# sea-sky-web/Vision-based-Spatio-Temporal-Analysis

Hardware: AMD Instinct MI355X
Metric: multi-cam frames/sec (7-cam→480×1440 BEV) (higher is better)
Workload: dtype f32; 1 GPU; 7-cam 1080x1920 -> resnet50(stride-8 features)+proj C=64 -> IPM warp -> mean -> 480x1440 BEV (BASELINE configs[1]); cameras=7, cameras_per_gpu=7, channels=64, bev_memory_format=NCHW, parallelism=frame-sharded x1 (no collective)

## Files before the change

### vision-based-spatio-temporal-analysis_amd/csrc/bev_conv_x6.hip

```cpp
#include <hip/hip_runtime.h>
#include <stdint.h>

#include <type_traits>

#include "../../include/bev_mi355x.h"
#include "bev_act.h"

namespace {

typedef __bf16 bf16x8 __attribute__((ext_vector_type(8)));
typedef __bf16 bf16x4 __attribute__((ext_vector_type(4)));
typedef float f32x16 __attribute__((ext_vector_type(16)));
typedef float f32x4 __attribute__((ext_vector_type(4)));
typedef unsigned u32x4 __attribute__((ext_vector_type(4)));
typedef unsigned u32x2 __attribute__((ext_vector_type(2)));

constexpr int XBK = 16;
constexpr int XROW = 24;

__device__ __attribute__((aligned(16))) float g_xzero4[4] = {0.f, 0.f, 0.f, 0.f};

__host__ __device__ inline int64_t kpad_x(int K) { return (K + XBK - 1) / XBK * XBK; }
__host__ __device__ inline int64_t copad_x(int Co) { return (Co + 127) / 128 * 128; }

// ... 650 lines not shown
        _Pragma("unroll") for (int i = 0; i < TM; ++i)                                                     \
            _Pragma("unroll") for (int p = 0; p < 3; ++p)                                                  \
                fa[i][p] = *(const bf16x8 *)(AS + p * APL + (wm * TM * 32 + i * 32 + r32) * YROW + 16 * (KK) + 8 * h); \
        _Pragma("unroll") for (int i = 0; i < TM; ++i)                                                     \
            _Pragma("unroll") for (int j = 0; j < TN; ++j) {                                               \
                acc[i][j] = __builtin_amdgcn_mfma_f32_32x32x16_bf16(fa[i][0], BC[j][0], acc[i][j], 0, 0, 0); \
                acc[i][j] = __builtin_amdgcn_mfma_f32_32x32x16_bf16(fa[i][0], BC[j][1], acc[i][j], 0, 0, 0); \
                acc[i][j] = __builtin_amdgcn_mfma_f32_32x32x16_bf16(fa[i][1], BC[j][0], acc[i][j], 0, 0, 0); \
                acc[i][j] = __builtin_amdgcn_mfma_f32_32x32x16_bf16(fa[i][0], BC[j][2], acc[i][j], 0, 0, 0); \
                acc[i][j] = __builtin_amdgcn_mfma_f32_32x32x16_bf16(fa[i][2], BC[j][0], acc[i][j], 0, 0, 0); \
                acc[i][j] = __builtin_amdgcn_mfma_f32_32x32x16_bf16(fa[i][1], BC[j][1], acc[i][j], 0, 0, 0); \
            }                                                                                              \
    } while (0)
#define X6B_MFMA(BUF, KS)                                                                                  \
    do {                                                                                                   \
        const __bf16 *As = lds + (BUF) * STAGE;                                                            \
        X6B_SLICE(As, 0, bs0);                                                                             \
        X6B_BLOAD(bs0, 2 * (KS) + 2);                                                                      \
        X6B_SLICE(As, 1, bs1);                                                                             \
    } while (0)

    const int nk = a.Kp / YBK;
    X6B_BLOAD(bs0, 0);
    X6B_GLOAD(va0);
    if (nk > 1) X6B_GLOAD(va1);
    X6B_SWRITE(0, va0);
    __syncthreads();
    int ks = 0;
    for (; ks + 3 < nk; ks += 2) {
        X6B_BLOAD(bs1, 2 * ks + 1);
        X6B_GLOAD(va0);
        X6B_MFMA(0, ks);
        X6B_SWRITE(1, va1);
        __syncthreads();
        X6B_BLOAD(bs1, 2 * ks + 3);
        X6B_GLOAD(va1);
        X6B_MFMA(1, ks + 1);
        X6B_SWRITE(0, va0);
        __syncthreads();
    }
    if (ks + 2 < nk) {
        X6B_BLOAD(bs1, 2 * ks + 1);
        X6B_GLOAD(va0);
        X6B_MFMA(0, ks);
        X6B_SWRITE(1, va1);
        __syncthreads();
        X6B_BLOAD(bs1, 2 * ks + 3);
        X6B_MFMA(1, ks + 1);
        X6B_SWRITE(0, va0);
        __syncthreads();
        X6B_BLOAD(bs1, 2 * ks + 5);
        X6B_MFMA(0, ks + 2);
    } else if (ks + 1 < nk) {
        X6B_BLOAD(bs1, 2 * ks + 1);
        X6B_MFMA(0, ks);
        X6B_SWRITE(1, va1);
        __syncthreads();
        X6B_BLOAD(bs1, 2 * ks + 3);
        X6B_MFMA(1, ks + 1);
    } else {
        X6B_BLOAD(bs1, 2 * ks + 1);
        X6B_MFMA(0, ks);
    }
#undef X6B_MFMA
#undef X6B_SLICE
#undef X6B_BLOAD
#undef X6B_SWRITE
#undef X6B_GLOAD
    if constexpr (CHAIN > 0) {
        x6_chain_epilogue<WM, WN, TM, TN, CHAIN == 2 ? 4 : 0>(a, lds_raw, acc, wave, lane, wm, wn, m0);
        return;
    }
    x6_epilogue<TM, TN>(a, (float *)lds_raw, acc, wave, lane, wn, wm, m0, n0);
}

template <int WM, int WN, int TM, int TN, int CHAIN = 0>
__global__ __launch_bounds__(256, CHAIN ? 2 : 3) void k_conv_x6s(ConvX a) {
    constexpr bool BLDS = CHAIN > 0;
    constexpr int BM = WM * TM * 32, BN = WN * TN * 32;
    constexpr int APL = BM * 32;
    constexpr int BST = BLDS ? BN / 32 * 6 * 512 : 0;
    constexpr int STAGE = 3 * APL + BST;
    constexpr int RW = BM / 4;
    constexpr int RG = RW / 16;
    constexpr int BPW = BLDS ? BN / 32 * 6 / 4 : 0;
    constexpr int EPIB = CHAIN ? x6_chain_lds_bytes<BM, BN>() : x6_epi_bytes<TN>();
    constexpr int LDSB = (2 * STAGE * 2 > EPIB) ? 2 * STAGE * 2 : EPIB;
    static_assert(RW % 16 == 0, "whole DMA groups per wave");
    static_assert(!BLDS || (BN / 32 * 6) % 4 == 0, "whole B pieces per wave");
    __shared__ __attribute__((aligned(16))) unsigned char lds_raw[LDSB];
    const __bf16 *lds = (const __bf16 *)lds_raw;

    const int tid = threadIdx.x;
    const int lane = tid & 63, wave = __builtin_amdgcn_readfirstlane(tid >> 6);
    const int wm = wave / WN, wn = wave % WN;
    const int n_tiles = (a.Co + BN - 1) / BN;
    unsigned bid = blockIdx.x;
    {
        const unsigned nb = gridDim.x, q = nb / 8, r = nb % 8, xc = bid % 8;
        bid = (xc < r ? xc * (q + 1) : r * (q + 1) + (xc - r) * q) + bid / 8;
    }
    const int64_t m0 = (int64_t)(bid / n_tiles) * BM;
    const int n0 = (bid % n_tiles) * BN;

    int64_t abase[RG];
    int aiy[RG], aix[RG];
    bool aok[RG];
#pragma unroll
    for (int g = 0; g < RG; ++g) {
        const int row = wave * RW + 16 * g + (lane >> 2);
        const int lc = (lane & 3) ^ ((row >> 2) & 3);
        const int64_t m = m0 + row;
        aok[g] = m < a.M;
        const int64_t mm = aok[g] ? m : 0;
        const int ox = (int)(mm % a.Wo);
        const int64_t t = mm / a.Wo;
        const int oy = (int)(t % a.Ho);
        const int64_t n = t / a.Ho;
        aiy[g] = oy * a.stride - a.pad;
        aix[g] = ox * a.stride - a.pad;
        abase[g] = ((n * a.H + aiy[g]) * a.W + aix[g]) * a.Ci + 8 * lc;
    }
    const unsigned lbase = (unsigned)__builtin_amdgcn_readfirstlane((int)lds_addr(lds_raw));
    const int S = a.Kp / XBK;
    int ky = 0, kx = 0, ci0 = 0, kstep = 0;
    const __bf16 *bsrc = a.wp + (int64_t)(n0 >> 5) * S * 1536 + lane * 8;
    auto issue = [&](int buf) {
        if constexpr (BLDS) {
            const unsigned db = lbase + (unsigned)(buf * STAGE * 2 + 3 * APL * 2);
#pragma unroll
            for (int i = 0; i < BPW; ++i) {
                const int q = wave + 4 * i, cbl = q / 6, r = q % 6;
                dma16(bsrc + ((int64_t)cbl * S + 2 * kstep + r / 3) * 1536 + (r % 3) * 512,
                      db + (unsigned)(q * 1024));
            }
            ++kstep;
        }
        const int64_t toff = ((int64_t)ky * a.dil * a.W + kx * a.dil) * a.Ci + ci0;
        const unsigned d0 = lbase + (unsigned)(buf * STAGE * 2) + (unsigned)(wave * RW * 64);
#pragma unroll
        for (int g = 0; g < RG; ++g) {
            const int iy = aiy[g] + ky * a.dil, ix = aix[g] + kx * a.dil;
            const bool in = aok[g] && (unsigned)iy < (unsigned)a.H && (unsigned)ix < (unsigned)a.W;
            const __bf16 *src = a.xs + abase[g] + toff;
#pragma unroll
            for (int p = 0; p < 3; ++p)
                dma16(in ? (const void *)(src + p * a.xps) : (const void *)g_xzero4,
                      d0 + (unsigned)(p * APL * 2 + g * 1024));
        }
        ci0 += YBK;
        if (ci0 == a.Ci) {
            ci0 = 0;
            if (++kx == a.KW) {
                kx = 0;
                ++ky;
            }
        }
    };

    const __amdgpu_buffer_rsrc_t rw = __builtin_amdgcn_make_buffer_rsrc(
        const_cast<__bf16 *>(a.wp), 0, (int)(uint32_t)(copad_x(a.Co) / 32 * (int64_t)S * 3072), 0x00020000);
    const int cb0 = (n0 + wn * TN * 32) >> 5;
    const int vl = lane * 16;
    bf16x8 bs0[TN][3], bs1[TN][3];
#define X6S_BLOAD(BS, G)                                                                                   \
    do {                                                                                                   \
        const int g_ = (G) < S ? (G) : S - 1;                                                              \
        _Pragma("unroll") for (int j = 0; j < TN; ++j)                                                     \
            _Pragma("unroll") for (int p = 0; p < 3; ++p)                                                  \
                BS[j][p] = __builtin_bit_cast(                                                             \
                    bf16x8, __builtin_amdgcn_raw_buffer_load_b128(rw, vl, (((cb0 + j) * S + g_) * 3 + p) * 1024, 0)); \
    } while (0)
    const int r32 = lane & 31, h = lane >> 5;
#define X6S_SLICE(AS, KK, BC)                                                                              \
    do {                                                                                                   \
        bf16x8 fa[TM][3];                                                                                  \
        _Pragma("unroll") for (int i = 0; i < TM; ++i) {                                                   \
            const int R = wm * TM * 32 + i * 32 + r32;                                                     \
            const int ph = (2 * (KK) + h) ^ ((R >> 2) & 3);                                                \
            _Pragma("unroll") for (int p = 0; p < 3; ++p)                                                  \
                fa[i][p] = *(const bf16x8 *)(AS + p * APL + R * 32 + ph * 8);                              \
        }                                                                                                  \
        _Pragma("unroll") for (int i = 0; i < TM; ++i)                                                     \
            _Pragma("unroll") for (int j = 0; j < TN; ++j) {                                               \
                acc[i][j] = __builtin_amdgcn_mfma_f32_32x32x16_bf16(fa[i][0], BC[j][0], acc[i][j], 0, 0, 0); \
                acc[i][j] = __builtin_amdgcn_mfma_f32_32x32x16_bf16(fa[i][0], BC[j][1], acc[i][j], 0, 0, 0); \
                acc[i][j] = __builtin_amdgcn_mfma_f32_32x32x16_bf16(fa[i][1], BC[j][0], acc[i][j], 0, 0, 0); \
                acc[i][j] = __builtin_amdgcn_mfma_f32_32x32x16_bf16(fa[i][0], BC[j][2], acc[i][j], 0, 0, 0); \
                acc[i][j] = __builtin_amdgcn_mfma_f32_32x32x16_bf16(fa[i][2], BC[j][0], acc[i][j], 0, 0, 0); \
                acc[i][j] = __builtin_amdgcn_mfma_f32_32x32x16_bf16(fa[i][1], BC[j][1], acc[i][j], 0, 0, 0); \
            }                                                                                              \
    } while (0)

    f32x16 acc[TM][TN];
#pragma unroll
    for (int i = 0; i < TM; ++i)
#pragma unroll
        for (int j = 0; j < TN; ++j) acc[i][j] = (f32x16){0};
    const int nk = a.Kp / YBK;
    if constexpr (BLDS) {
        issue(0);
        asm volatile("s_waitcnt vmcnt(0)" ::: "memory");
        __syncthreads();
        for (int ks = 0; ks < nk; ++ks) {
            const int cur = ks & 1;
            if (ks + 1 < nk) issue(cur ^ 1);
            const __bf16 *As = lds + cur * STAGE;
            const __bf16 *Bs = As + 3 * APL + lane * 8;
#pragma unroll
            for (int kk = 0; kk < 2; ++kk) {
                bf16x8 fb[TN][3];
#pragma unroll
                for (int j = 0; j < TN; ++j)
#pragma unroll
                    for (int p = 0; p < 3; ++p) fb[j][p] = *(const bf16x8 *)(Bs + (((wn * TN + j) * 2 + kk) * 3 + p) * 512);
                X6S_SLICE(As, kk, fb);
            }
            asm volatile("s_waitcnt vmcnt(0)" ::: "memory");
            __syncthreads();
        }
    } else {
        X6S_BLOAD(bs0, 0);
        issue(0);
        asm volatile("s_waitcnt vmcnt(0)" ::: "memory");
        __syncthreads();
        for (int ks = 0; ks < nk; ++ks) {
            const int cur = ks & 1;
            if (ks + 1 < nk) issue(cur ^ 1);
            const __bf16 *As = lds + cur * STAGE;
            X6S_BLOAD(bs1, 2 * ks + 1);
            X6S_SLICE(As, 0, bs0);
            X6S_BLOAD(bs0, 2 * ks + 2);
            X6S_SLICE(As, 1, bs1);
            asm volatile("s_waitcnt vmcnt(0)" ::: "memory");
            __syncthreads();
        }
    }
#undef X6S_SLICE
#undef X6S_BLOAD
    if constexpr (CHAIN > 0) {
        x6_chain_epilogue<WM, WN, TM, TN, CHAIN == 2 ? 4 : 0>(a, lds_raw, acc, wave, lane, wm, wn, m0);
        return;
    }
    x6_epilogue<TM, TN>(a, (float *)lds_raw, acc, wave, lane, wn, wm, m0, n0);
}

__global__ void k_split3(const float *__restrict__ x, int64_t n, __bf16 *__restrict__ out) {
    const int64_t t = (int64_t)blockIdx.x * blockDim.x + threadIdx.x;
    if (t >= n) return;
    __bf16 h, m, l;
    split3(x[t], h, m, l);
    out[t] = h;
    out[t + n] = m;
    out[t + 2 * n] = l;
}

template <int BM, int BN>
int launch_x6(void (*kernel)(ConvX), const ConvX &a, hipStream_t st) {
    const int64_t blocks = ((a.M + BM - 1) / BM) * ((a.Co + BN - 1) / BN);
    if (blocks >= ((int64_t)1 << 31)) return BEV_ERR_ARGS;
    hipLaunchKernelGGL(kernel, dim3((unsigned)blocks), dim3(256), 0, st, a);
    return (int)hipGetLastError();
}

ConvX conv_x6_args(const float *x, const uint16_t *packed, const float *bias, const float *res, float *y, int N, int H,
                   int W, int Ci, int Co, int KH, int KW, int stride, int pad, int dil, int Ho, int Wo, int act,
                   int ldy) {
    ConvX a;
    a.x = x, a.wp = (const __bf16 *)packed, a.bias = bias, a.res = res, a.y = y;
    a.N = N, a.H = H, a.W = W, a.Ci = Ci, a.Co = Co, a.KH = KH, a.KW = KW, a.stride = stride, a.pad = pad;
    a.dil = dil, a.Ho = Ho, a.Wo = Wo, a.act = act, a.ldy = ldy;
    a.Kp = (int)kpad_x(Ci * KH * KW);
    a.M = (int64_t)N * Ho * Wo;
    return a;
}

int g_x6_tile = 0;
int g_x6_nt = 0;
int g_x6_kernel = 0;

template <bool DUAL>
int dispatch_x6(const ConvX &a0, hipStream_t st) {
    ConvX a = a0;
    a.nta = g_x6_nt;
    const int t = g_x6_tile ? g_x6_tile : (a.Co <= 64 ? 2 : 1);
    if (!DUAL && a.xs) {
        if (t == 2) return launch_x6<128, 64>(k_conv_x6s<4, 1, 1, 2>, a, st);
        return launch_x6<128, 128>(k_conv_x6s<2, 2, 2, 2>, a, st);
    }
    const bool wide = a.Ci % YBK == 0 && (!DUAL || a.Ci2 % YBK == 0) && g_x6_kernel != 1;
    if (wide) {
        if (t == 2 && !DUAL && a.nta) return launch_x6<128, 64>(k_conv_x6b<4, 1, 1, 2, false, 0, true>, a, st);
        if (t == 2) return launch_x6<128, 64>(k_conv_x6b<4, 1, 1, 2, DUAL>, a, st);
        return launch_x6<128, 128>(k_conv_x6b<2, 2, 2, 2, DUAL>, a, st);
    }
    if (t == 2) return launch_x6<128, 64>(k_conv_x6<4, 1, 1, 2, DUAL>, a, st);
    return launch_x6<128, 128>(k_conv_x6<2, 2, 2, 2, DUAL>, a, st);
}

namespace stem6 {
constexpr int TW = 64, TH = 8, NTHR = 512;
constexpr int PR = 2 * TH + 5;
constexpr int PC = 2 * TW + 5;
constexpr int PP = 80;
constexpr int RP = 2 * PP, CP = PR * RP, PATCH = 3 * CP;
constexpr int NE = 3 * PR * PC;
constexpr int PER_T = (NE + NTHR - 1) / NTHR;
constexpr int NS = 10;
constexpr int WB = 2 * NS * 3 * 512;
__host__ __device__ constexpr int koff(int k) {
    return k >= 147 ? 0 : (k % 3) * CP + (k / 21) * RP + (((k / 3) % 7) & 1) * PP + (((k / 3) % 7) >> 1);
}
}

struct StemX6Args {
    const float *__restrict__ x;
    const __bf16 *__restrict__ wp;
    const float *__restrict__ bias;
    float *__restrict__ y;
    int H, W, Co, Ho, Wo, relu, nTx, nTy;
    int64_t ntiles;
    float *__restrict__ edge_b, *__restrict__ edge_r;
    int Hp, Wp;
};

__device__ __forceinline__ void stem6_fetch(const StemX6Args &a, int64_t t, int tid, float (&pv)[stem6::PER_T]) {
    using namespace stem6;
    const int tx = (int)(t % a.nTx);
    const int64_t r_ = t / a.nTx;
    const int ty = (int)(r_ % a.nTy);
    const int64_t img = r_ / a.nTy;
    const int row0 = 2 * ty * TH - 3, col0 = 2 * tx * TW - 3;
    const float *xi = a.x + img * 3 * (int64_t)a.H * a.W;
#pragma unroll
    for (int i = 0; i < PER_T; ++i) {
        const int e = tid + NTHR * i;
        const int cr = e / PC, c = e - cr * PC;
        const int ci = cr / PR, r = cr - ci * PR;
        const int gy = row0 + r, gx = col0 + c;
        const bool in = e < NE && gy >= 0 && gy < a.H && gx >= 0 && gx < a.W;
        pv[i] = *(in ? xi + ((int64_t)ci * a.H + gy) * a.W + gx : (const float *)g_xzero4);
    }
}

__device__ __forceinline__ void stem6_put(float *pl, int tid, const float (&pv)[stem6::PER_T]) {
    using namespace stem6;
#pragma unroll
    for (int i = 0; i < PER_T; ++i) {
        const int e = tid + NTHR * i;
        if (e < NE) {
            const int cr = e / PC, c = e - cr * PC;
            const int ci = cr / PR, r = cr - ci * PR;
            const int o = ci * CP + r * RP + (c & 1) * PP + (c >> 1);
            __bf16 hh, mm, ll;
            split3(pv[i], hh, mm, ll);
            reinterpret_cast<unsigned *>(pl)[o] = (unsigned)__builtin_bit_cast(unsigned short, hh) |
                                                  ((unsigned)__builtin_bit_cast(unsigned short, mm) << 16);
            reinterpret_cast<__bf16 *>(pl + PATCH)[o] = ll;
        }
    }
}

__device__ __forceinline__ float pool_mx(float m, float v) { return max_nan(m, v); }

template <bool POOL>
__global__ __launch_bounds__(stem6::NTHR, 1) void k_stem_x6(StemX6Args a) {
    using namespace stem6;
    __shared__ __attribute__((aligned(16))) unsigned char lds_raw[WB * 2 + PATCH * 6];
    __bf16 *wl = (__bf16 *)lds_raw;
    float *pl = (float *)(lds_raw + WB * 2);
    const int tid = threadIdx.x, lane = tid & 63, wave = tid >> 6, h = lane >> 5, r32 = lane & 31;
    for (int e = tid; e < WB / 8; e += NTHR) reinterpret_cast<u32x4 *>(wl)[e] = reinterpret_cast<const u32x4 *>(a.wp)[e];
    float pv[PER_T];
    int64_t t = blockIdx.x;
    stem6_fetch(a, t < a.ntiles ? t : 0, tid, pv);
    stem6_put(pl, tid, pv);
    __syncthreads();

    const float *P = pl + wave * 2 * RP + r32;
    const __bf16 *PL = reinterpret_cast<const __bf16 *>(pl + PATCH) + wave * 2 * RP + r32;
    const float b0 = (r32 < a.Co) ? a.bias[r32] : 0.0f;
    const float b1 = (32 + r32 < a.Co) ? a.bias[32 + r32] : 0.0f;
    for (; t < a.ntiles; t += gridDim.x) {
        const int64_t tn = t + gridDim.x;
        stem6_fetch(a, tn < a.ntiles ? tn : t, tid, pv);
        f32x16 acc[2][2];
#pragma unroll
        for (int i = 0; i < 2; ++i)
#pragma unroll
            for (int j = 0; j < 2; ++j) acc[i][j] = (f32x16){0};
#pragma unroll
        for (int sl = 0; sl < NS; ++sl) {
            int hv = h;
            asm volatile("" : "+v"(hv));
            const __bf16 *wlb = wl + lane * 8;
            asm volatile("" : "+v"(wlb));
            bf16x8 fb[2][3];
#pragma unroll
            for (int j = 0; j < 2; ++j)
#pragma unroll
                for (int p = 0; p < 3; ++p)
                    fb[j][p] = *(const bf16x8 *)(wlb + ((j * NS + sl) * 3 + p) * 512);
#pragma unroll
            for (int mt = 0; mt < 2; ++mt) {
                bf16x8 fa[3];
#pragma unroll
                for (int e = 0; e < 8; ++e) {
                    const int o0 = koff(16 * sl + e), o1 = koff(16 * sl + 8 + e);
                    const int o = 32 * mt + (hv ? o1 : o0);
                    const unsigned hm = reinterpret_cast<const unsigned *>(P)[o];
                    fa[0][e] = __builtin_bit_cast(__bf16, (unsigned short)(hm & 0xffffu));
                    fa[1][e] = __builtin_bit_cast(__bf16, (unsigned short)(hm >> 16));
                    fa[2][e] = PL[o];
                }
#pragma unroll
                for (int j = 0; j < 2; ++j) {
                    f32x16 &c = acc[mt][j];
                    c = __builtin_amdgcn_mfma_f32_32x32x16_bf16(fa[0], fb[j][0], c, 0, 0, 0);
                    c = __builtin_amdgcn_mfma_f32_32x32x16_bf16(fa[0], fb[j][1], c, 0, 0, 0);
                    c = __builtin_amdgcn_mfma_f32_32x32x16_bf16(fa[1], fb[j][0], c, 0, 0, 0);
                    c = __builtin_amdgcn_mfma_f32_32x32x16_bf16(fa[0], fb[j][2], c, 0, 0, 0);
                    c = __builtin_amdgcn_mfma_f32_32x32x16_bf16(fa[2], fb[j][0], c, 0, 0, 0);
                    c = __builtin_amdgcn_mfma_f32_32x32x16_bf16(fa[1], fb[j][1], c, 0, 0, 0);
                }
            }
            __builtin_amdgcn_sched_barrier(0);
        }
        if constexpr (POOL) {
            const int tx = (int)(t % a.nTx);
            const int64_t r_ = t / a.nTx;
            const int ty = (int)(r_ % a.nTy);
            const int64_t img = r_ / a.nTy;
            const int oy = ty * TH + wave;
            const int oxb = tx * TW;
            float hp[2][4][2][2];
            float pa3[2][2][4];
            float c63[2];
#pragma unroll
            for (int mt = 0; mt < 2; ++mt)
#pragma unroll
                for (int j = 0; j < 2; ++j)
#pragma unroll
                    for (int b = 0; b < 4; ++b) {
                        float v[4];
#pragma unroll
                        for (int u = 0; u < 4; ++u) {
                            const int ox = oxb + 32 * mt + 8 * b + 4 * h + u;
                            const float z = acc[mt][j][4 * b + u] + (j ? b1 : b0);
                            v[u] = oy < a.Ho && ox < a.Wo ? relu_f(z) : 0.0f;
                        }
                        pa3[mt][j][b] = __shfl_xor(v[3], 32);
                        hp[mt][b][1][j] = pool_mx(pool_mx(v[1], v[2]), v[3]);
                        hp[mt][b][0][j] = pool_mx(v[0], v[1]);
                        if (mt == 1 && b == 3) c63[j] = v[3];
                    }
#pragma unroll
            for (int mt = 0; mt < 2; ++mt)
#pragma unroll
                for (int j = 0; j < 2; ++j)
#pragma unroll
                    for (int b = 0; b < 4; ++b) {
                        const float prev0 = b > 0 ? pa3[mt][j][b - 1] : (mt > 0 ? pa3[mt - 1][j][3] : 0.0f);
                        hp[mt][b][0][j] = pool_mx(hp[mt][b][0][j], h ? pa3[mt][j][b] : prev0);
                    }
            __syncthreads();
            float *xl = pl;
            if (wave & 1) {
                float *o = xl + (wave >> 1) * 34 * 64 + lane;
#pragma unroll
                for (int mt = 0; mt < 2; ++mt)
#pragma unroll
                    for (int b = 0; b < 4; ++b)
#pragma unroll
                        for (int pc = 0; pc < 2; ++pc)
#pragma unroll
                            for (int j = 0; j < 2; ++j) o[(((mt * 4 + b) * 2 + pc) * 2 + j) * 64] = hp[mt][b][pc][j];
                o[32 * 64] = c63[0];
                o[33 * 64] = c63[1];
            }
            __syncthreads();
            const int64_t tile = t;
            if (wave == TH - 1) {
                float *eb = a.edge_b + tile * (32 * 64);
#pragma unroll
                for (int mt = 0; mt < 2; ++mt)
#pragma unroll
                    for (int b = 0; b < 4; ++b)
#pragma unroll
                        for (int pc = 0; pc < 2; ++pc)
#pragma unroll
                            for (int j = 0; j < 2; ++j)
                                eb[(16 * mt + 4 * b + 2 * h + pc) * 64 + r32 + 32 * j] = hp[mt][b][pc][j];
                if (h) {
                    a.edge_r[(tile * 5 + 4) * 64 + r32] = c63[0];
                    a.edge_r[(tile * 5 + 4) * 64 + 32 + r32] = c63[1];
                }
            } else if (!(wave & 1)) {
                const int p = wave >> 1;
                const float *up = xl + (p - 1) * 34 * 64 + lane, *dn = xl + p * 34 * 64 + lane;
#pragma unroll
                for (int mt = 0; mt < 2; ++mt)
#pragma unroll
                    for (int b = 0; b < 4; ++b)
#pragma unroll
                        for (int pc = 0; pc < 2; ++pc)
#pragma unroll
                            for (int j = 0; j < 2; ++j) {
                                const int e = (((mt * 4 + b) * 2 + pc) * 2 + j) * 64;
                                float m = pool_mx(hp[mt][b][pc][j], dn[e]);
                                if (p > 0) m = pool_mx(m, up[e]);
                                hp[mt][b][pc][j] = m;
                            }
                float e0 = pool_mx(c63[0], dn[32 * 64]), e1 = pool_mx(c63[1], dn[33 * 64]);
                if (p > 0) {
                    e0 = pool_mx(e0, up[32 * 64]);
                    e1 = pool_mx(e1, up[33 * 64]);
                }
                if (h) {
                    a.edge_r[(tile * 5 + p) * 64 + r32] = e0;
                    a.edge_r[(tile * 5 + p) * 64 + 32 + r32] = e1;
                }
                const int prow = ty * (TH / 2) + p;
                if (prow < a.Hp) {
                    float *yr = a.y + ((img * a.Hp + prow) * (int64_t)a.Wp) * 64;
#pragma unroll
                    for (int mt = 0; mt < 2; ++mt)
#pragma unroll
                        for (int b = 0; b < 4; ++b)
#pragma unroll
                            for (int pc = 0; pc < 2; ++pc) {
                                const int Q = tx * (TW / 2) + 16 * mt + 4 * b + 2 * h + pc;
                                if (Q < a.Wp) {
                                    yr[(int64_t)Q * 64 + r32] = hp[mt][b][pc][0];
                                    yr[(int64_t)Q * 64 + 32 + r32] = hp[mt][b][pc][1];
                                }
                            }
                }
            }
        } else {
            const int tx = (int)(t % a.nTx);
            const int64_t r_ = t / a.nTx;
            const int ty = (int)(r_ % a.nTy);
            const int64_t img = r_ / a.nTy;
            const int oy = ty * TH + wave;
            const int oxb = tx * TW;
            if (oy < a.Ho) {
                float *yr = a.y + ((img * a.Ho + oy) * (int64_t)a.Wo) * a.Co;
#pragma unroll
                for (int mt = 0; mt < 2; ++mt)
#pragma unroll
                    for (int r = 0; r < 16; ++r) {
                        const int ox = oxb + 32 * mt + (r & 3) + 8 * (r >> 2) + 4 * h;
                        if (ox < a.Wo) {
                            float v0 = acc[mt][0][r] + b0, v1 = acc[mt][1][r] + b1;
                            if (a.relu) {
                                v0 = relu_f(v0);
                                v1 = relu_f(v1);
                            }
                            float *yp = yr + (int64_t)ox * a.Co;
                            if (r32 < a.Co) yp[r32] = v0;
                            if (32 + r32 < a.Co) yp[32 + r32] = v1;
                        }
                    }
            }
        }
        __syncthreads();
        stem6_put(pl, tid, pv);
        __syncthreads();
    }
}

__global__ __launch_bounds__(256) void k_stem_pool_seams(float *__restrict__ y, const float *__restrict__ edge_b,
                                                         const float *__restrict__ edge_r, int nTx, int nTy,
                                                         int64_t ntiles, int Hp, int Wp) {
    const int64_t g = (int64_t)blockIdx.x * 256 + threadIdx.x;
    const int64_t tile = g / (35 * 16);
    if (tile >= ntiles) return;
    const int k = (int)(g - tile * (35 * 16)), s = k >> 4, c4 = k & 15;
    const int tx = (int)(tile % nTx);
    const int64_t r_ = tile / nTx;
    const int ty = (int)(r_ % nTy);
    const int64_t img = r_ / nTy;
    const int p = s < 32 ? 0 : s - 31, q = s < 32 ? s : 0;
    const int P = ty * (stem6::TH / 2) + p, Q = tx * (stem6::TW / 2) + q;
    if (P >= Hp || Q >= Wp || (p == 0 && ty == 0 && (q > 0 || tx == 0))) return;
    float4 *yp = reinterpret_cast<float4 *>(y + (((img * Hp + P) * (int64_t)Wp + Q) * 64)) + c4;
    float4 m = *yp;
    auto mx = [](float4 a, float4 b) {
        return make_float4(pool_mx(a.x, b.x), pool_mx(a.y, b.y), pool_mx(a.z, b.z), pool_mx(a.w, b.w));
    };
    if (p == 0 && ty > 0) m = mx(m, reinterpret_cast<const float4 *>(edge_b + ((tile - nTx) * 32 + q) * 64)[c4]);
    if (q == 0 && tx > 0) {
        m = mx(m, reinterpret_cast<const float4 *>(edge_r + ((tile - 1) * 5 + p) * 64)[c4]);
        if (p == 0 && ty > 0)
            m = mx(m, reinterpret_cast<const float4 *>(edge_r + ((tile - nTx - 1) * 5 + 4) * 64)[c4]);
    }
    *yp = m;
}

}

namespace bev {
int conv_x6_tune(int knob, int value) {
    int *slot = knob == BEV_TUNE_CONV_X6_TILE ? &g_x6_tile : knob == BEV_TUNE_CONV_X6_NT ? &g_x6_nt : &g_x6_kernel;
    if (value < 0 || value > (knob == BEV_TUNE_CONV_X6_TILE ? 2 : 1)) return BEV_ERR_ARGS;
    const int old = *slot;
    *slot = value;
    return old;
}
}

extern "C" {

int64_t bev_conv_packed_size_x6(int Co, int Ci, int KH, int KW) {
    if (Co <= 0 || Ci <= 0 || KH <= 0 || KW <= 0) return BEV_ERR_ARGS;
    return copad_x(Co) * kpad_x(Ci * KH * KW) * 3;
}

int bev_conv_pack_weights_x6(const float *w, int Co, int Ci, int KH, int KW, uint16_t *packed, void *stream) {
    if (!w || !packed || Co <= 0 || Ci <= 0 || KH <= 0 || KW <= 0) return BEV_ERR_ARGS;
    const int64_t Kp = kpad_x(Ci * KH * KW), Cop = copad_x(Co), n = Kp * Cop;
    hipLaunchKernelGGL(k_pack_x6, dim3((unsigned)((n + 255) / 256)), dim3(256), 0, (hipStream_t)stream, w, Co, Ci, KH,
                       KW, Kp, Cop, (__bf16 *)packed);
    return (int)hipGetLastError();
}

int bev_conv2d_x6_f32(const float *x, const uint16_t *xs, int N, int H, int W, int Ci, const uint16_t *packed,
                      const float *bias, const float *residual, int Co, int KH, int KW, int stride, int pad,
                      int dilation, int act, float *y, uint16_t *ys, int ldy, int Ho, int Wo, void *stream) {
    if ((!x == !xs) || !packed || (!y == !ys) || N < 0 || H <= 0 || W <= 0 || Ci <= 0 || Co <= 0 || KH <= 0 ||
        KW <= 0 || stride <= 0 || pad < 0 || dilation <= 0 || act < 0 || act > 2 || ldy < Co)
        return BEV_ERR_ARGS;
    if (Ci % (xs ? YBK : XBK) != 0) return BEV_ERR_ARGS;
    if (Ho != (H + 2 * pad - dilation * (KH - 1) - 1) / stride + 1 ||
        Wo != (W + 2 * pad - dilation * (KW - 1) - 1) / stride + 1 || Ho <= 0 || Wo <= 0)
        return BEV_ERR_ARGS;
    if ((((uintptr_t)x | (uintptr_t)xs | (uintptr_t)packed) & 15) != 0) return BEV_ERR_ARGS;
    if (residual && ldy != Co) return BEV_ERR_ARGS;
    if (ys && (ldy != Co || Co % 4 != 0 || ((uintptr_t)ys & 7) != 0)) return BEV_ERR_ARGS;
    if (N == 0) return 0;
    ConvX a = conv_x6_args(x, packed, bias, residual, y, N, H, W, Ci, Co, KH, KW, stride, pad, dilation, Ho, Wo, act,
                           ldy);
    a.xs = (const __bf16 *)xs;
    a.ys = (__bf16 *)ys;
    a.xps = (int64_t)N * H * W * Ci;
    a.yps = a.M * Co;
    return dispatch_x6<false>(a, (hipStream_t)stream);
}

int bev_split3_f32(const float *x, int64_t n, uint16_t *planes, void *stream) {
    if (!x || !planes || n < 0) return BEV_ERR_ARGS;
    if (n == 0) return 0;
    hipLaunchKernelGGL(k_split3, dim3((unsigned)((n + 255) / 256)), dim3(256), 0, (hipStream_t)stream, x, n,
                       (__bf16 *)planes);
    return (int)hipGetLastError();
}

int bev_conv2d_dual_x6_f32(const float *x, int N, int Ho, int Wo, int Ci, const float *x2, int H2, int W2, int Ci2,
                           int stride2, const uint16_t *packed, const float *bias, int Co, int act, float *y,
                           void *stream) {
    if (!x || !x2 || !packed || !y || N < 0 || Ho <= 0 || Wo <= 0 || Ci <= 0 || Ci2 <= 0 || H2 <= 0 || W2 <= 0 ||
        stride2 <= 0 || Co <= 0 || act < 0 || act > 2)
        return BEV_ERR_ARGS;
    if (Ci % XBK != 0 || Ci2 % XBK != 0) return BEV_ERR_ARGS;
    if (Ho != (H2 - 1) / stride2 + 1 || Wo != (W2 - 1) / stride2 + 1) return BEV_ERR_ARGS;
    if ((((uintptr_t)x | (uintptr_t)x2 | (uintptr_t)packed) & 15) != 0) return BEV_ERR_ARGS;
    if (N == 0) return 0;
    ConvX a = conv_x6_args(x, packed, bias, nullptr, y, N, Ho, Wo, Ci, Co, 1, 1, 1, 0, 1, Ho, Wo, act, Co);
    a.Kp = (int)kpad_x(Ci + Ci2);
    a.x2 = x2;
    a.Ci2 = Ci2, a.H2 = H2, a.W2 = W2, a.stride2 = stride2;
    return dispatch_x6<true>(a, (hipStream_t)stream);
}

int bev_conv2d_chain_x6_f32(const float *x, const uint16_t *xs, int N, int H, int W, int Ci,
                            const uint16_t *packed, const float *bias, int Co, int KH, int KW, int stride, int pad,
                            int act, const uint16_t *packed2, const float *bias2, int Co2, const float *residual,
                            int act2, float *y, int Ho, int Wo, void *stream) {
    if ((!x == !xs) || !packed || !packed2 || !y || N < 0 || H <= 0 || W <= 0 || KH <= 0 || KW <= 0 ||
        stride <= 0 || pad < 0 || act < 0 || act > 2 || act2 < 0 || act2 > 2)
        return BEV_ERR_ARGS;
    if (Ci % YBK != 0 || (Co != 64 && Co != 128) || Co2 <= 0 || Co2 % 64 != 0 ||
        (((uintptr_t)x | (uintptr_t)xs | (uintptr_t)packed | (uintptr_t)packed2) & 15) != 0)
        return BEV_ERR_ARGS;
    if (Ho != (H + 2 * pad - KH) / stride + 1 || Wo != (W + 2 * pad - KW) / stride + 1 || Ho <= 0 || Wo <= 0)
        return BEV_ERR_ARGS;
    if (N == 0) return 0;
    ConvX a = conv_x6_args(x, packed, bias, residual, y, N, H, W, Ci, Co, KH, KW, stride, pad, 1, Ho, Wo, act, Co2);
    a.xs = (const __bf16 *)xs;
    a.xps = (int64_t)N * H * W * Ci;
    a.wp2 = (const __bf16 *)packed2;
    a.bias2 = bias2;
    a.Co2 = Co2, a.act2 = act2;
    if (Co != 64 && Co2 % 128 != 0) return BEV_ERR_ARGS;
    const hipStream_t st = (hipStream_t)stream;
    if (xs) {
        if (Co == 64) return launch_x6<128, 64>(k_conv_x6s<4, 1, 1, 2, 1>, a, st);
        return launch_x6<64, 128>(k_conv_x6s<2, 2, 1, 2, 1>, a, st);
    }
    if (Co == 64) return launch_x6<128, 64>(k_conv_x6b<4, 1, 1, 2, false, 1>, a, st);
    return launch_x6<64, 128>(k_conv_x6b<2, 2, 1, 2, false, 1>, a, st);
}

int bev_conv2d_chain_dual_x6_f32(const float *x, const uint16_t *xs, int N, int H, int W, int Ci,
                                 const uint16_t *packed, const float *bias, int Co, int KH, int KW, int stride,
                                 int pad, int act, const float *x2, int H2, int W2, int Ci2, int stride2,
                                 const uint16_t *packed2, const float *bias2, int Co2, int act2, float *y, int Ho,
                                 int Wo, void *stream) {
    if ((!x == !xs) || !x2 || !packed || !packed2 || !y || N < 0 || H <= 0 || W <= 0 || KH <= 0 || KW <= 0 ||
        stride <= 0 || pad < 0 || act < 0 || act > 2 || act2 < 0 || act2 > 2 || stride2 <= 0 || H2 <= 0 || W2 <= 0)
        return BEV_ERR_ARGS;
    if (Ci % YBK != 0 || Co != 64 || Ci2 != 64 || Co2 <= 0 || Co2 % 64 != 0 ||
        (((uintptr_t)x | (uintptr_t)xs | (uintptr_t)x2 | (uintptr_t)packed | (uintptr_t)packed2) & 15) != 0)
        return BEV_ERR_ARGS;
    if (Ho != (H + 2 * pad - KH) / stride + 1 || Wo != (W + 2 * pad - KW) / stride + 1 || Ho <= 0 || Wo <= 0 ||
        Ho != (H2 - 1) / stride2 + 1 || Wo != (W2 - 1) / stride2 + 1)
        return BEV_ERR_ARGS;
    if (N == 0) return 0;
    ConvX a = conv_x6_args(x, packed, bias, nullptr, y, N, H, W, Ci, Co, KH, KW, stride, pad, 1, Ho, Wo, act, Co2);
    a.x2 = x2;
    a.Ci2 = Ci2, a.H2 = H2, a.W2 = W2, a.stride2 = stride2;
    a.xs = (const __bf16 *)xs;
    a.xps = (int64_t)N * H * W * Ci;
    a.wp2 = (const __bf16 *)packed2;
    a.bias2 = bias2;
    a.Co2 = Co2, a.act2 = act2;
    if (xs) return launch_x6<128, 64>(k_conv_x6s<4, 1, 1, 2, 2>, a, (hipStream_t)stream);
    return launch_x6<128, 64>(k_conv_x6b<4, 1, 1, 2, false, 2>, a, (hipStream_t)stream);
}

int bev_conv2d_stem_x6_f32(const float *x, int N, int H, int W, const uint16_t *packed, const float *bias, int Co,
                           int relu, float *y, int Ho, int Wo, void *stream) {
    if (!x || !packed || !bias || !y || N <= 0 || H <= 0 || W <= 0 || Co <= 0 || Co > 64 ||
        Ho != (H + 6 - 7) / 2 + 1 || Wo != (W + 6 - 7) / 2 + 1 || (((uintptr_t)packed) & 15) != 0)
        return BEV_ERR_ARGS;
    static int num_cu = 0;
    if (num_cu == 0) {
        int dev = 0, n = 0;
        if (hipGetDevice(&dev) != hipSuccess ||
            hipDeviceGetAttribute(&n, hipDeviceAttributeMultiprocessorCount, dev) != hipSuccess || n <= 0)
            n = 256;
        num_cu = n;
    }
    StemX6Args a;
    a.x = x;
    a.wp = (const __bf16 *)packed;
    a.bias = bias;
    a.y = y;
    a.H = H, a.W = W, a.Co = Co, a.Ho = Ho, a.Wo = Wo, a.relu = relu;
    a.nTx = (Wo + stem6::TW - 1) / stem6::TW;
    a.nTy = (Ho + stem6::TH - 1) / stem6::TH;
    a.ntiles = (int64_t)N * a.nTx * a.nTy;
    a.edge_b = a.edge_r = nullptr;
    a.Hp = a.Wp = 0;
    const int64_t grid = a.ntiles < num_cu ? a.ntiles : num_cu;
    hipLaunchKernelGGL(k_stem_x6<false>, dim3((unsigned)grid), dim3(stem6::NTHR), 0, (hipStream_t)stream, a);
    return (int)hipGetLastError();
}

int64_t bev_conv2d_stem_pool_x6_workspace(int N, int H, int W) {
    if (N <= 0 || H <= 0 || W <= 0) return BEV_ERR_ARGS;
    const int Ho = (H + 6 - 7) / 2 + 1, Wo = (W + 6 - 7) / 2 + 1;
    const int64_t nt = (int64_t)N * ((Wo + stem6::TW - 1) / stem6::TW) * ((Ho + stem6::TH - 1) / stem6::TH);
    return nt * (32 + 5) * 64 * (int64_t)sizeof(float);
}

int bev_conv2d_stem_pool_x6_f32(const float *x, int N, int H, int W, const uint16_t *packed, const float *bias,
                                int Co, float *y, int Hp, int Wp, void *workspace, int64_t workspace_bytes,
                                void *stream) {
    const int Ho = (H + 6 - 7) / 2 + 1, Wo = (W + 6 - 7) / 2 + 1;
    if (!x || !packed || !bias || !y || !workspace || N <= 0 || H <= 0 || W <= 0 || Co != 64 ||
        Hp != (Ho + 2 - 3) / 2 + 1 || Wp != (Wo + 2 - 3) / 2 + 1 || (((uintptr_t)packed | (uintptr_t)y |
                                                                       (uintptr_t)workspace) & 15) != 0)
        return BEV_ERR_ARGS;
    if (workspace_bytes < bev_conv2d_stem_pool_x6_workspace(N, H, W)) return BEV_ERR_ARGS;
    static int num_cu = 0;
    if (num_cu == 0) {
        int dev = 0, n = 0;
        if (hipGetDevice(&dev) != hipSuccess ||
            hipDeviceGetAttribute(&n, hipDeviceAttributeMultiprocessorCount, dev) != hipSuccess || n <= 0)
            n = 256;
        num_cu = n;
    }
    StemX6Args a;
    a.x = x;
    a.wp = (const __bf16 *)packed;
    a.bias = bias;
    a.y = y;
    a.H = H, a.W = W, a.Co = Co, a.Ho = Ho, a.Wo = Wo, a.relu = 1;
    a.nTx = (Wo + stem6::TW - 1) / stem6::TW;
    a.nTy = (Ho + stem6::TH - 1) / stem6::TH;
    a.ntiles = (int64_t)N * a.nTx * a.nTy;
    a.edge_b = (float *)workspace;
    a.edge_r = a.edge_b + a.ntiles * 32 * 64;
    a.Hp = Hp, a.Wp = Wp;
    const int64_t grid = a.ntiles < num_cu ? a.ntiles : num_cu;
    hipLaunchKernelGGL(k_stem_x6<true>, dim3((unsigned)grid), dim3(stem6::NTHR), 0, (hipStream_t)stream, a);
    const int64_t nthr = a.ntiles * 35 * 16;
    hipLaunchKernelGGL(k_stem_pool_seams, dim3((unsigned)((nthr + 255) / 256)), dim3(256), 0, (hipStream_t)stream, y,
                       a.edge_b, a.edge_r, a.nTx, a.nTy, a.ntiles, Hp, Wp);
    return (int)hipGetLastError();
}

}
```

Before: 135.7 frames/s.

## Restructure stem conv LDS patch into row-run planes with vector A-fragment loads

```diff
diff --git a/vision-based-spatio-temporal-analysis_amd/csrc/bev_conv_x6.hip b/vision-based-spatio-temporal-analysis_amd/csrc/bev_conv_x6.hip
--- a/vision-based-spatio-temporal-analysis_amd/csrc/bev_conv_x6.hip
+++ b/vision-based-spatio-temporal-analysis_amd/csrc/bev_conv_x6.hip
@@ -976,15 +976,16 @@
 constexpr int TW = 64, TH = 8, NTHR = 512;
 constexpr int PR = 2 * TH + 5;
 constexpr int PC = 2 * TW + 5;
-constexpr int PP = 80;
-constexpr int RP = 2 * PP, CP = PR * RP, PATCH = 3 * CP;
-constexpr int NE = 3 * PR * PC;
-constexpr int PER_T = (NE + NTHR - 1) / NTHR;
-constexpr int NS = 10;
+constexpr int PITCH = 136;
+constexpr int PLANE = 3 * PR * PITCH;
+constexpr int PER_T = 17;
+constexpr int NRUN = 3 * 7;
+constexpr int NS = (NRUN + 2) / 2;
 constexpr int WB = 2 * NS * 3 * 512;
-__host__ __device__ constexpr int koff(int k) {
-    return k >= 147 ? 0 : (k % 3) * CP + (k / 21) * RP + (((k / 3) % 7) & 1) * PP + (((k / 3) % 7) >> 1);
-}
+constexpr int S_PANEL = 10;
+__host__ __device__ constexpr int roff(int run) { return run >= NRUN ? 0 : ((run % 3) * PR + run / 3) * PITCH; }
+static_assert(PITCH >= 2 * TW + 6 && PITCH % 2 == 0, "slot 7 of the last output column inside the row");
+static_assert(4 * 34 * 64 * 4 <= 3 * PLANE * 2, "the pool epilogue's row exchange fits in the patch");
 }
 
 struct StemX6Args {
@@ -998,7 +999,7 @@
     int Hp, Wp;
 };
 
-__device__ __forceinline__ void stem6_fetch(const StemX6Args &a, int64_t t, int tid, float (&pv)[stem6::PER_T]) {
+__device__ __forceinline__ unsigned stem6_fetch(const StemX6Args &a, int64_t t, int tid, float (&pv)[stem6::PER_T]) {
     using namespace stem6;
     const int tx = (int)(t % a.nTx);
     const int64_t r_ = t / a.nTx;
@@ -1006,31 +1007,33 @@
     const int64_t img = r_ / a.nTy;
     const int row0 = 2 * ty * TH - 3, col0 = 2 * tx * TW - 3;
     const float *xi = a.x + img * 3 * (int64_t)a.H * a.W;
+    unsigned in = 0;
 #pragma unroll
     for (int i = 0; i < PER_T; ++i) {
-        const int e = tid + NTHR * i;
-        const int cr = e / PC, c = e - cr * PC;
-        const int ci = cr / PR, r = cr - ci * PR;
+        const int cr = i < PER_T - 1 ? (tid >> 7) + 4 * i : tid >> 3;
+        const int c = i < PER_T - 1 ? (tid & 127) : 2 * TW + (tid & 7);
+        const int ci = (cr >= PR) + (cr >= 2 * PR), r = cr - ci * PR;
         const int gy = row0 + r, gx = col0 + c;
-        const bool in = e < NE && gy >= 0 && gy < a.H && gx >= 0 && gx < a.W;
-        pv[i] = *(in ? xi + ((int64_t)ci * a.H + gy) * a.W + gx : (const float *)g_xzero4);
-    }
-}
-
-__device__ __forceinline__ void stem6_put(float *pl, int tid, const float (&pv)[stem6::PER_T]) {
+        const bool ok = cr < 3 * PR && c < PC && (unsigned)gy < (unsigned)a.H && (unsigned)gx < (unsigned)a.W;
+        pv[i] = xi[ok ? ((int64_t)ci * a.H + gy) * a.W + gx : 0];
+        in |= (unsigned)ok << i;
+    }
+    return in;
+}
+
+__device__ __forceinline__ void stem6_put(__bf16 *pl, int tid, const float (&pv)[stem6::PER_T], unsigned in) {
     using namespace stem6;
+    __bf16 *q = pl + (tid >> 7) * PITCH + (tid & 127);
 #pragma unroll
     for (int i = 0; i < PER_T; ++i) {
-        const int e = tid + NTHR * i;
-        if (e < NE) {
-            const int cr = e / PC, c = e - cr * PC;
-            const int ci = cr / PR, r = cr - ci * PR;
-            const int o = ci * CP + r * RP + (c & 1) * PP + (c >> 1);
+        const bool last = i == PER_T - 1;
+        if (last ? (tid >> 3) < 3 * PR && (tid & 7) < PC - 2 * TW : i < PER_T - 2 || (tid >> 7) < 3 * PR - 4 * i) {
+            __bf16 *o = last ? pl + (tid >> 3) * PITCH + 2 * TW + (tid & 7) : q + 4 * i * PITCH;
             __bf16 hh, mm, ll;
-            split3(pv[i], hh, mm, ll);
-            reinterpret_cast<unsigned *>(pl)[o] = (unsigned)__builtin_bit_cast(unsigned short, hh) |
-                                                  ((unsigned)__builtin_bit_cast(unsigned short, mm) << 16);
-            reinterpret_cast<__bf16 *>(pl + PATCH)[o] = ll;
+            split3((in >> i) & 1u ? pv[i] : 0.0f, hh, mm, ll);
+            o[0] = hh;
+            o[PLANE] = mm;
+            o[2 * PLANE] = ll;
         }
     }
 }
@@ -1040,24 +1043,32 @@
 template <bool POOL>
 __global__ __launch_bounds__(stem6::NTHR, 1) void k_stem_x6(StemX6Args a) {
     using namespace stem6;
-    __shared__ __attribute__((aligned(16))) unsigned char lds_raw[WB * 2 + PATCH * 6];
+    __shared__ __attribute__((aligned(16))) unsigned char lds_raw[WB * 2 + 3 * PLANE * 2];
     __bf16 *wl = (__bf16 *)lds_raw;
-    float *pl = (float *)(lds_raw + WB * 2);
+    __bf16 *pl = (__bf16 *)(lds_raw + WB * 2);
     const int tid = threadIdx.x, lane = tid & 63, wave = tid >> 6, h = lane >> 5, r32 = lane & 31;
-    for (int e = tid; e < WB / 8; e += NTHR) reinterpret_cast<u32x4 *>(wl)[e] = reinterpret_cast<const u32x4 *>(a.wp)[e];
+    for (int f = tid; f < WB / 8; f += NTHR) {
+        const int ln = f & 63, fr = f >> 6, p = fr % 3, sl = (fr / 3) % NS, cb = fr / (3 * NS);
+        const int run = 2 * sl + (ln >> 5), ky = run / 3, ci = run - 3 * ky, n = 32 * cb + (ln & 31);
+        const unsigned short *src = reinterpret_cast<const unsigned short *>(a.wp);
+        unsigned w[8];
+#pragma unroll
+        for (int kx = 0; kx < 7; ++kx)
+            w[kx] = run < NRUN ? (unsigned)src[frag_index(n, (ky * 7 + kx) * 3 + ci, p, S_PANEL)] : 0u;
+        reinterpret_cast<u32x4 *>(wl)[f] = (u32x4){w[0] | (w[1] << 16), w[2] | (w[3] << 16), w[4] | (w[5] << 16), w[6]};
+    }
     float pv[PER_T];
     int64_t t = blockIdx.x;
-    stem6_fetch(a, t < a.ntiles ? t : 0, tid, pv);
-    stem6_put(pl, tid, pv);
+    unsigned pin = stem6_fetch(a, t < a.ntiles ? t : 0, tid, pv);
+    stem6_put(pl, tid, pv, pin);
     __syncthreads();
 
-    const float *P = pl + wave * 2 * RP + r32;
-    const __bf16 *PL = reinterpret_cast<const __bf16 *>(pl + PATCH) + wave * 2 * RP + r32;
+    const __bf16 *P = pl + wave * 2 * PITCH + 2 * r32;
     const float b0 = (r32 < a.Co) ? a.bias[r32] : 0.0f;
     const float b1 = (32 + r32 < a.Co) ? a.bias[32 + r32] : 0.0f;
     for (; t < a.ntiles; t += gridDim.x) {
         const int64_t tn = t + gridDim.x;
-        stem6_fetch(a, tn < a.ntiles ? tn : t, tid, pv);
+        pin = stem6_fetch(a, tn < a.ntiles ? tn : t, tid, pv);
         f32x16 acc[2][2];
 #pragma unroll
         for (int i = 0; i < 2; ++i)
@@ -1067,8 +1078,10 @@
         for (int sl = 0; sl < NS; ++sl) {
             int hv = h;
             asm volatile("" : "+v"(hv));
-            const __bf16 *wlb = wl + lane * 8;
-            asm volatile("" : "+v"(wlb));
+            const __bf16 *Pr = P + (hv ? roff(2 * sl + 1) : roff(2 * sl));
+            int wo = lane * 8;
+            asm volatile("" : "+v"(wo));
+            const __bf16 *wlb = wl + wo;
             bf16x8 fb[2][3];
 #pragma unroll
             for (int j = 0; j < 2; ++j)
@@ -1079,13 +1092,9 @@
             for (int mt = 0; mt < 2; ++mt) {
                 bf16x8 fa[3];
 #pragma unroll
-                for (int e = 0; e < 8; ++e) {
-                    const int o0 = koff(16 * sl + e), o1 = koff(16 * sl + 8 + e);
-                    const int o = 32 * mt + (hv ? o1 : o0);
-                    const unsigned hm = reinterpret_cast<const unsigned *>(P)[o];
-                    fa[0][e] = __builtin_bit_cast(__bf16, (unsigned short)(hm & 0xffffu));
-                    fa[1][e] = __builtin_bit_cast(__bf16, (unsigned short)(hm >> 16));
-                    fa[2][e] = PL[o];
+                for (int p = 0; p < 3; ++p) {
+                    const unsigned *q = reinterpret_cast<const unsigned *>(Pr + p * PLANE + 64 * mt);
+                    fa[p] = __builtin_bit_cast(bf16x8, (u32x4){q[0], q[1], q[2], q[3] & 0xffffu});
                 }
 #pragma unroll
                 for (int j = 0; j < 2; ++j) {
@@ -1138,7 +1147,7 @@
                         hp[mt][b][0][j] = pool_mx(hp[mt][b][0][j], h ? pa3[mt][j][b] : prev0);
                     }
             __syncthreads();
-            float *xl = pl;
+            float *xl = reinterpret_cast<float *>(pl);
             if (wave & 1) {
                 float *o = xl + (wave >> 1) * 34 * 64 + lane;
 #pragma unroll
@@ -1153,6 +1162,18 @@
                 o[33 * 64] = c63[1];
             }
             __syncthreads();
+            const int p = wave >> 1;
+            float uv[34], dv[34];
+            if (!(wave & 1)) {
+                const float *up = xl + (p > 0 ? p - 1 : p) * 34 * 64 + lane, *dn = xl + p * 34 * 64 + lane;
+#pragma unroll
+                for (int e = 0; e < 34; ++e) {
+                    dv[e] = dn[e * 64];
+                    uv[e] = up[e * 64];
+                }
+            }
+            __syncthreads();
+            stem6_put(pl, tid, pv, pin);
             const int64_t tile = t;
             if (wave == TH - 1) {
                 float *eb = a.edge_b + tile * (32 * 64);
@@ -1170,8 +1191,6 @@
                     a.edge_r[(tile * 5 + 4) * 64 + 32 + r32] = c63[1];
                 }
             } else if (!(wave & 1)) {
-                const int p = wave >> 1;
-                const float *up = xl + (p - 1) * 34 * 64 + lane, *dn = xl + p * 34 * 64 + lane;
 #pragma unroll
                 for (int mt = 0; mt < 2; ++mt)
 #pragma unroll
@@ -1180,15 +1199,14 @@
                         for (int pc = 0; pc < 2; ++pc)
 #pragma unroll
                             for (int j = 0; j < 2; ++j) {
-                                const int e = (((mt * 4 + b) * 2 + pc) * 2 + j) * 64;
-                                float m = pool_mx(hp[mt][b][pc][j], dn[e]);
-                                if (p > 0) m = pool_mx(m, up[e]);
-                                hp[mt][b][pc][j] = m;
+                                const int e = ((mt * 4 + b) * 2 + pc) * 2 + j;
+                                const float m = pool_mx(hp[mt][b][pc][j], dv[e]);
+                                hp[mt][b][pc][j] = p > 0 ? pool_mx(m, uv[e]) : m;
                             }
-                float e0 = pool_mx(c63[0], dn[32 * 64]), e1 = pool_mx(c63[1], dn[33 * 64]);
+                float e0 = pool_mx(c63[0], dv[32]), e1 = pool_mx(c63[1], dv[33]);
                 if (p > 0) {
-                    e0 = pool_mx(e0, up[32 * 64]);
-                    e1 = pool_mx(e1, up[33 * 64]);
+                    e0 = pool_mx(e0, uv[32]);
+                    e1 = pool_mx(e1, uv[33]);
                 }
                 if (h) {
                     a.edge_r[(tile * 5 + p) * 64 + r32] = e0;
@@ -1218,6 +1236,8 @@
             const int64_t img = r_ / a.nTy;
             const int oy = ty * TH + wave;
             const int oxb = tx * TW;
+            __syncthreads();
+            stem6_put(pl, tid, pv, pin);
             if (oy < a.Ho) {
                 float *yr = a.y + ((img * a.Ho + oy) * (int64_t)a.Wo) * a.Co;
 #pragma unroll
@@ -1238,8 +1258,6 @@
                     }
             }
         }
-        __syncthreads();
-        stem6_put(pl, tid, pv);
         __syncthreads();
     }
 }
```

Result: faster. 137.9 frames/s, median of 6 (+1.6%).
